# svohr/mixemt

Hardware: AMD Instinct MI355X
Metric: read x hap cells/sec through the EM iteration (EM iters/sec reported beside it as em_iters_per_s), 1000000 reads x 5408 haps in total, whole job (higher is better)
Workload: dtype f64

## Files before the change

### mixemt_amd/csrc/coded_kernels.hpp

```cpp
#ifndef MIXEMT_CODED_KERNELS_HPP
#define MIXEMT_CODED_KERNELS_HPP

#define ENC_THREADS 256
#define ENC_SLOTS 1024
#define ENC_MAX_CODES 256
#define ENC_MAX_WIDE 1024
#define ENC_WIDE_SLOTS 4096
#define ENC_EMPTY 0xFFFFFFFFFFFFFFFFull

__host__ __device__ __forceinline__ int rec_code_bytes(int nd, int ldc) { return nd > ENC_MAX_CODES ? 2 * ldc : ldc; }
__device__ __forceinline__ int rec_code_at(const uint8_t *codes, int h, bool wide) {
    return wide ? (int)reinterpret_cast<const uint16_t *>(codes)[h] : (int)codes[h];
}

template <int NCH, bool WIDE>
__device__ __forceinline__ void encode_one_row(int64_t r, const double *__restrict__ M, int64_t ldm, int H, int ldc,
                                               uint8_t *__restrict__ rec, int64_t rec_cap, int64_t *__restrict__ rec_off,
                                               int32_t *__restrict__ ndist, double *__restrict__ rowmax,
                                               unsigned long long *__restrict__ stats) {
    constexpr int NW = ENC_THREADS / 64;
    constexpr int SLOTS = WIDE ? ENC_WIDE_SLOTS : ENC_SLOTS;
    constexpr int MAXC = WIDE ? ENC_MAX_WIDE : ENC_MAX_CODES;
    constexpr int SPT = SLOTS / ENC_THREADS;
    __shared__ unsigned long long s_key[SLOTS];
// ... 212 lines not shown
                                               int64_t n_list = 0, const int32_t *__restrict__ nquad = nullptr, int vbid = -1,
                                               int vgrid = 0) {
    static_assert(NBUF >= 3, "codes NBUF - 1 rows ahead, tables NBUF - 2");
    constexpr int NW = THREADS / 64;
    constexpr int AUX = NT ? 2 : 0;
    __shared__ double s_tbl[NBUF][ENC_MAX_CODES];
    __shared__ __attribute__((aligned(16))) double red[NBUF][NW];
    const int t = threadIdx.x, lane = t & 63, wv = t >> 6;
    const int nword = ldc >> 2;
    const int64_t bid = vbid >= 0 ? (int64_t)vbid : (int64_t)blockIdx.x, grid = vbid >= 0 ? (int64_t)vgrid : (int64_t)gridDim.x;
    const row_deal deal(row_list != nullptr ? n_list : R, bid, grid);
    const int voff = t * 4;
    int last_w = t + (NCH - 1) * THREADS;
    if (last_w > nword - 1) last_w = nword - 1;
    const int voff_last = last_w * 4;
    const bool tbl_thread = (THREADS <= ENC_MAX_CODES) || t < ENC_MAX_CODES;
    const int tslot = t & (ENC_MAX_CODES - 1);
    typedef unsigned int u2v __attribute__((ext_vector_type(2)));
    __shared__ int s_chk[2];
    if constexpr (CHECK) {
        if (t == 0) s_chk[0] = s_chk[1] = 0;
        __syncthreads();
    }
    auto list_row = [&](int64_t e) -> int64_t {
        int64_t r = wide_rows[e];
        if constexpr (CHECK) {
            if (r < 0 || r >= R || (e > 0 && wide_rows[e - 1] >= r)) {
                s_chk[1] = 1;
                r = -1;
            }
        }
        return r;
    };
    auto list_nd = [&](int64_t r) -> int {
        if (r < 0) return 0;
        int nd = ndist[r];
        if constexpr (CHECK) {
            if (nd <= ENC_MAX_CODES) {
                s_chk[1] = 1;
                nd = 0;
            }
        }
        return nd;
    };

    __shared__ long long s_off[2][THREADS];
    __shared__ double s_wr[2][THREADS];
    __shared__ int s_nd[2][THREADS];
    auto fetch_meta = [&](int half, int64_t q0) {
        const int64_t q = q0 + t;
        int64_t r = deal.row(q);
        bool struck = false;
        if (row_list != nullptr) {
            const int64_t e = r;
            r = row_list[e];
            if constexpr (CHECK) {
                if (r < 0 || r >= R || (e > 0 && row_list[e - 1] >= r)) {
                    s_chk[1] = 1;
                    r = 0;
                    struck = true;
                }
            }
        }
        int nd = ndist[r];
        if (nd > ENC_MAX_CODES) {
            if constexpr (CHECK) {
                if (row_list != nullptr) s_chk[1] = 1;
                else if (deal.live(q)) atomicAdd(&s_chk[0], 1);
            }
            nd = 0;
        }
        if constexpr (CHECK) {
            if (row_list != nullptr && !struck && (nd <= 0 || nquad[r] != 0)) {
                s_chk[1] = 1;
                struck = true;
            }
        }
        if (struck) nd = 0;
        s_off[half][t] = rec_off[r];
        s_nd[half][t] = nd;
        s_wr[half][t] = (deal.live(q) && nd > 0) ? (w != nullptr ? w[r] : 1.0) : 0.0;
    };

    unsigned int cw[NBUF][NCH];
    double tring[NBUF];
    int pre_off_lo, pre_off_hi, pre_nd;
    double pre_wr;
    auto read_meta = [&](int64_t q_load, int64_t q_weight) {
        const int half = (int)((q_load / THREADS) & 1), idx = (int)(q_load % THREADS);
        const long long off = s_off[half][idx];
        pre_nd = __builtin_amdgcn_readfirstlane(s_nd[half][idx]);
        pre_off_hi = __builtin_amdgcn_readfirstlane((int)(off >> 32));
        pre_off_lo = __builtin_amdgcn_readfirstlane((int)off);
        pre_wr = s_wr[(q_weight / THREADS) & 1][q_weight % THREADS];
    };
    auto load_row = [&](unsigned int(&cws)[NCH], double &tbl_entry) {
        const int nd = pre_nd;
        const uint8_t *base = rec + (((long long)pre_off_hi << 32) | (unsigned int)pre_off_lo);
        const auto rs = __builtin_amdgcn_make_buffer_rsrc(const_cast<uint8_t *>(base), 0, ldc, 0x00020000);
#pragma unroll
        for (int k = 0; k < NCH - 1; ++k) cws[k] = __builtin_amdgcn_raw_buffer_load_b32(rs, voff, k * THREADS * 4, AUX);
        cws[NCH - 1] = __builtin_amdgcn_raw_buffer_load_b32(rs, voff_last, 0, AUX);
        if (tbl_thread) {
            const auto rt = __builtin_amdgcn_make_buffer_rsrc(const_cast<uint8_t *>(base + ldc), 0, nd * 8, 0x00020000);
            const u2v v = __builtin_amdgcn_raw_buffer_load_b64(rt, tslot * 8, 0, AUX);
            tbl_entry = __hiloint2double((int)v.y, (int)v.x);
        }
    };

    const unsigned int three = 3;
    auto entry_off = [&](unsigned int word, auto E) -> unsigned int {
        constexpr int e = decltype(E)::value;
        unsigned int r;
        if constexpr (e == 0) asm("v_lshlrev_b32_sdwa %0, %1, %2 dst_sel:DWORD dst_unused:UNUSED_PAD src0_sel:DWORD src1_sel:BYTE_0" : "=v"(r) : "v"(three), "v"(word));
        else if constexpr (e == 1) asm("v_lshlrev_b32_sdwa %0, %1, %2 dst_sel:DWORD dst_unused:UNUSED_PAD src0_sel:DWORD src1_sel:BYTE_1" : "=v"(r) : "v"(three), "v"(word));
        else if constexpr (e == 2) asm("v_lshlrev_b32_sdwa %0, %1, %2 dst_sel:DWORD dst_unused:UNUSED_PAD src0_sel:DWORD src1_sel:BYTE_2" : "=v"(r) : "v"(three), "v"(word));
        else asm("v_lshlrev_b32_sdwa %0, %1, %2 dst_sel:DWORD dst_unused:UNUSED_PAD src0_sel:DWORD src1_sel:BYTE_3" : "=v"(r) : "v"(three), "v"(word));
        return r;
    };
    auto lookup = [&](const char *tb, unsigned int word, auto E) -> double {
        return *reinterpret_cast<const double *>(tb + entry_off(word, E));
    };
    using E0 = std::integral_constant<int, 0>;
    using E1 = std::integral_constant<int, 1>;
    using E2 = std::integral_constant<int, 2>;
    using E3 = std::integral_constant<int, 3>;

    double v[NCH][4];
    auto lookup_row = [&](const char *tb, const unsigned int(&cws)[NCH]) {
#pragma unroll
        for (int k = 0; k < NCH; ++k) {
            v[k][0] = lookup(tb, cws[k], E0{});
            v[k][1] = lookup(tb, cws[k], E1{});
            v[k][2] = lookup(tb, cws[k], E2{});
            v[k][3] = lookup(tb, cws[k], E3{});
        }
    };

    auto step = [&](auto J, int64_t q) {
        constexpr int j = decltype(J)::value;
        constexpr int jn = (j + 1) % NBUF, jl = (j + NBUF - 1) % NBUF;
        if constexpr (!RESIDENT) {
            if ((q % THREADS) == 0) fetch_meta((int)((q / THREADS + 1) & 1), q + THREADS);
        }
        load_row(cw[jl], tring[jl]);
        const double wr = pre_wr;
        double s4[4] = {0.0, 0.0, 0.0, 0.0};
#pragma unroll
        for (int k = 0; k < NCH; ++k)
#pragma unroll
            for (int e = 0; e < 4; ++e) s4[e] = fma(v[k][e], p[k][e], s4[e]);
        double s = (s4[0] + s4[1]) + (s4[2] + s4[3]);
        __builtin_amdgcn_s_setprio(1);
        s = wave_sum_lane63(s);
        if (lane == 63) red[j][wv] = s;
        if (tbl_thread) s_tbl[jn][tslot] = tring[jn];
        __syncthreads();
        read_meta(q + NBUF, q + 1);
        static_assert(NW == 4, "four wave sums");
        typedef double d2v __attribute__((ext_vector_type(2)));
        const d2v ra = *reinterpret_cast<const d2v *>(&red[j][0]), rb = *reinterpret_cast<const d2v *>(&red[j][2]);
        const double cf = readlane_f64(weight_over_norm(wr, (ra.x + ra.y) + (rb.x + rb.y)), 0);
        __builtin_amdgcn_s_setprio(0);
        const char *tbn = reinterpret_cast<const char *>(&s_tbl[jn][0]);
        auto upd = [&](int k, auto E) {
            constexpr int e = decltype(E)::value;
            acc[k][e] = fma(cf, v[k][e], acc[k][e]);
            asm volatile("" : "+v"(acc[k][e]));
            v[k][e] = lookup(tbn, cw[jn][k], E);
        };
#pragma unroll
        for (int k = 0; k < NCH; ++k) {
            upd(k, E0{});
            upd(k, E1{});
            upd(k, E2{});
            upd(k, E3{});
        }
    };

    const int64_t nq_w = (n_wide > bid) ? (n_wide - bid + grid - 1) / grid : 0;
    const bool wide_fetch = WIDE_PREFETCH && nq_w > 0 && (!RESIDENT || !meta_ready);
    int64_t w_row = -1;
    if (wide_fetch && t < nq_w) w_row = list_row(bid + (int64_t)t * grid);
    long long w_off = 0;
    int w_nd = CHECK ? -1 : 0;
    double w_wr = 0.0;

    if (deal.nq > 0) {
        if (!RESIDENT || !meta_ready) {
            __syncthreads();
            fetch_meta(0, 0);
            if constexpr (RESIDENT) fetch_meta(1, THREADS);
        }
        __syncthreads();
#pragma unroll
        for (int j = 0; j < NBUF - 1; ++j) {
            read_meta(j, 0);
            load_row(cw[j], tring[j]);
        }
        if (tbl_thread) s_tbl[0][tslot] = tring[0];
        __syncthreads();
        read_meta(NBUF - 1, 0);
        lookup_row(reinterpret_cast<const char *>(&s_tbl[0][0]), cw[0]);
        if (w_row >= 0) {
            w_off = rec_off[w_row];
            w_nd = ndist[w_row];
            w_wr = (w != nullptr) ? w[w_row] : 1.0;
        }
        for (int64_t q = 0; q < deal.nq; q += NBUF) {
            step(std::integral_constant<int, 0>{}, q);
            step(std::integral_constant<int, 1>{}, q + 1);
            step(std::integral_constant<int, 2>{}, q + 2);
            if constexpr (NBUF > 3) step(std::integral_constant<int, 3>{}, q + 3);
            if constexpr (NBUF > 4) step(std::integral_constant<int, 4>{}, q + 4);
            if constexpr (NBUF > 5) step(std::integral_constant<int, 5>{}, q + 5);
            static_assert(NBUF <= 6, "unrolled by hand");
        }
    }

    else if (w_row >= 0) {
        w_off = rec_off[w_row];
        w_nd = ndist[w_row];
        w_wr = (w != nullptr) ? w[w_row] : 1.0;
    }

    if (nq_w > 0) {
        __shared__ double s_wide[ENC_MAX_WIDE];
        __shared__ long long s_woff[THREADS];
        __shared__ double s_wwr[THREADS];
        __shared__ int s_wnd[THREADS];
        constexpr int TPT = ENC_MAX_WIDE / THREADS;
        const int voff8 = t * 8;
        const int voff8_last = last_w * 8;
        for (int64_t q0 = 0; q0 < nq_w; q0 += THREADS) {
            if (q0 == 0 && wide_fetch) {
                __syncthreads();
                if constexpr (CHECK) {
                    if (w_nd >= 0 && w_nd <= ENC_MAX_CODES) s_chk[1] = 1;
                    if (w_nd <= ENC_MAX_CODES) {
                        w_nd = 0;
                        w_wr = 0.0;
                    }
                }
                s_woff[t] = w_off;
                s_wnd[t] = w_nd;
                s_wwr[t] = w_wr;
            } else if (q0 > 0 || !RESIDENT || !meta_ready || nq_w > THREADS) {
                __syncthreads();
                const int64_t q = q0 + t;
                if (q < nq_w) {
                    const int64_t r = list_row(bid + q * grid);
                    const int nd = list_nd(r);
                    s_woff[t] = (r >= 0) ? rec_off[r] : 0;
                    s_wnd[t] = nd;
                    s_wwr[t] = (nd > 0) ? ((w != nullptr) ? w[r] : 1.0) : 0.0;
                }
            }
            __syncthreads();
            const int n_here = (int)((nq_w - q0) < THREADS ? (nq_w - q0) : THREADS);
            u2v cwa[NCH], cwb[NCH], cwc[NCH];
            double tna[TPT], tnb[TPT], tnc[TPT];
            auto fetch_wide = [&](int i, u2v(&cwn)[NCH], double(&tn)[TPT]) {
                const long long off = s_woff[i];
                const int nd = __builtin_amdgcn_readfirstlane(s_wnd[i]);
                const uint8_t *base = rec + (((long long)__builtin_amdgcn_readfirstlane((int)(off >> 32)) << 32) |
                                             (unsigned int)__builtin_amdgcn_readfirstlane((int)off));
                const auto rs = __builtin_amdgcn_make_buffer_rsrc(const_cast<uint8_t *>(base), 0, 2 * ldc, 0x00020000);
#pragma unroll
                for (int k = 0; k < NCH - 1; ++k) cwn[k] = __builtin_amdgcn_raw_buffer_load_b64(rs, voff8, k * THREADS * 8, AUX);
                cwn[NCH - 1] = __builtin_amdgcn_raw_buffer_load_b64(rs, voff8_last, 0, AUX);
                const auto rt = __builtin_amdgcn_make_buffer_rsrc(const_cast<uint8_t *>(base + 2 * ldc), 0, nd * 8, 0x00020000);
#pragma unroll
                for (int j = 0; j < TPT; ++j) {
                    const u2v x = __builtin_amdgcn_raw_buffer_load_b64(rt, (t + j * THREADS) * 8, 0, AUX);
                    tn[j] = __hiloint2double((int)x.y, (int)x.x);
                }
            };
            auto process_wide = [&](int i, const u2v(&cwn)[NCH], const double(&tn)[TPT]) {
                const double wr = s_wwr[i];
#pragma unroll
                for (int j = 0; j < TPT; ++j) s_wide[t + j * THREADS] = tn[j];
                __syncthreads();
                const char *tb = reinterpret_cast<const char *>(&s_wide[0]);
                double s4[4] = {0.0, 0.0, 0.0, 0.0};
#pragma unroll
                for (int k = 0; k < NCH; ++k) {
                    v[k][0] = *reinterpret_cast<const double *>(tb + ((cwn[k].x & 0xffffu) << 3));
                    v[k][1] = *reinterpret_cast<const double *>(tb + ((cwn[k].x >> 16) << 3));
                    v[k][2] = *reinterpret_cast<const double *>(tb + ((cwn[k].y & 0xffffu) << 3));
                    v[k][3] = *reinterpret_cast<const double *>(tb + ((cwn[k].y >> 16) << 3));
                }
#pragma unroll
                for (int k = 0; k < NCH; ++k)
#pragma unroll
                    for (int e = 0; e < 4; ++e) s4[e] = fma(v[k][e], p[k][e], s4[e]);
                double s = (s4[0] + s4[1]) + (s4[2] + s4[3]);
                s = wave_sum_lane63(s);
                if (lane == 63) red[0][wv] = s;
                __syncthreads();
                static_assert(NW == 4, "four wave sums");
                const double cf = readlane_f64(weight_over_norm(wr, (red[0][0] + red[0][1]) + (red[0][2] + red[0][3])), 0);
#pragma unroll
                for (int k = 0; k < NCH; ++k)
#pragma unroll
                    for (int e = 0; e < 4; ++e) acc[k][e] = fma(cf, v[k][e], acc[k][e]);
            };
            fetch_wide(0, cwa, tna);
// ... 180 lines not shown
```

### mixemt_amd/csrc/common.hpp

```cpp
#ifndef MIXEMT_COMMON_HPP
#define MIXEMT_COMMON_HPP

typedef double d2 __attribute__((ext_vector_type(2)));

#define MXM_MAX_WG 1024
#define MXM_MAX_BT 4

struct mxm_slots {
    int s[MXM_MAX_BT];
};
#define MXM_LINEAR_MIN_H 65

static thread_local char g_err[512] = "";

static int fail(int code, const char *fmt, const char *a = "", long long b = 0, long long c = 0) {
    snprintf(g_err, sizeof(g_err), fmt, a, b, c);
    return code;
}
#define HIP_TRY(expr)                                                                        \
    do {                                                                                     \
        hipError_t e_ = (expr);                                                              \
        if (e_ != hipSuccess) return fail(-2, "HIP error: %s (line %lld)", hipGetErrorString(e_), __LINE__); \
    } while (0)

#define MXM_MAX_DEVICES 64
static std::atomic<int> g_num_cu[MXM_MAX_DEVICES];
static int num_cu() {
    int dev = 0;
    if (hipGetDevice(&dev) != hipSuccess) return 256;
    const bool cached = dev >= 0 && dev < MXM_MAX_DEVICES;
    if (cached) {
        const int have = g_num_cu[dev].load(std::memory_order_relaxed);
        if (have > 0) return have;
    }
    hipDeviceProp_t prop;
    if (hipGetDeviceProperties(&prop, dev) != hipSuccess) return 256;
    const int n = prop.multiProcessorCount > 0 ? prop.multiProcessorCount : 256;
    if (cached) g_num_cu[dev].store(n, std::memory_order_relaxed);
    return n;
}

__device__ __forceinline__ double wave_sum(double v) {
#pragma unroll
    for (int off = 32; off > 0; off >>= 1) v += __shfl_xor(v, off, 64);
    return v;
}
__device__ __forceinline__ double wave_max(double v) {
#pragma unroll
    for (int off = 32; off > 0; off >>= 1) v = fmax(v, __shfl_xor(v, off, 64));
    return v;
}

template <int THREADS, bool IS_MAX>
__device__ __forceinline__ double block_reduce(double v, double *scratch) {
    constexpr int NW = THREADS / 64;
    v = IS_MAX ? wave_max(v) : wave_sum(v);
    __syncthreads();
    if ((threadIdx.x & 63) == 0) scratch[threadIdx.x >> 6] = v;
    __syncthreads();
    double r = scratch[0];
#pragma unroll
    for (int i = 1; i < NW; ++i) r = IS_MAX ? fmax(r, scratch[i]) : r + scratch[i];
    return r;
}

template <int CTRL>
__device__ __forceinline__ double dpp_mov_f64(double v) {
    int lo = __double2loint(v), hi = __double2hiint(v);
    lo = __builtin_amdgcn_mov_dpp(lo, CTRL, 0xf, 0xf, true);
    hi = __builtin_amdgcn_mov_dpp(hi, CTRL, 0xf, 0xf, true);
    return __hiloint2double(hi, lo);
}
__device__ __forceinline__ double readlane_f64(double v, int src_lane) {
    const int lo = __builtin_amdgcn_readlane(__double2loint(v), src_lane);
    const int hi = __builtin_amdgcn_readlane(__double2hiint(v), src_lane);
    return __hiloint2double(hi, lo);
}
template <int CTRL, int ROW_MASK>
__device__ __forceinline__ double dpp_mov_old_f64(double old, double v) {
    int lo = __double2loint(v), hi = __double2hiint(v);
    lo = __builtin_amdgcn_update_dpp(__double2loint(old), lo, CTRL, ROW_MASK, 0xf, false);
    hi = __builtin_amdgcn_update_dpp(__double2hiint(old), hi, CTRL, ROW_MASK, 0xf, false);
    return __hiloint2double(hi, lo);
}
__device__ __forceinline__ double wave_sum_lane63(double v) {
    v += dpp_mov_f64<0xB1>(v);
    v += dpp_mov_f64<0x4E>(v);
    v += dpp_mov_f64<0x141>(v);
    v += dpp_mov_f64<0x140>(v);
    v += dpp_mov_old_f64<0x142, 0xA>(0.0, v);
    v += dpp_mov_old_f64<0x143, 0xC>(0.0, v);
    return v;
}
__device__ __forceinline__ double swap32_add(double x, double y) {
    typedef unsigned int u2s __attribute__((ext_vector_type(2)));
    const u2s lo = __builtin_amdgcn_permlane32_swap((unsigned)__double2loint(x), (unsigned)__double2loint(y), false, false);
    const u2s hi = __builtin_amdgcn_permlane32_swap((unsigned)__double2hiint(x), (unsigned)__double2hiint(y), false, false);
    return __hiloint2double((int)hi.x, (int)lo.x) + __hiloint2double((int)hi.y, (int)lo.y);
}
__device__ __forceinline__ double swap16_add(double x, double y) {
    typedef unsigned int u2s __attribute__((ext_vector_type(2)));
    const u2s lo = __builtin_amdgcn_permlane16_swap((unsigned)__double2loint(x), (unsigned)__double2loint(y), false, false);
    const u2s hi = __builtin_amdgcn_permlane16_swap((unsigned)__double2hiint(x), (unsigned)__double2hiint(y), false, false);
    return __hiloint2double((int)hi.x, (int)lo.x) + __hiloint2double((int)hi.y, (int)lo.y);
}
__device__ __forceinline__ double wave_sum3_by_row(double a, double b, double c) {
    const double ab = swap32_add(a, b);
    const double cc = swap32_add(c, c);
    double v = swap16_add(ab, cc);
    v += dpp_mov_f64<0xB1>(v);
    v += dpp_mov_f64<0x4E>(v);
    v += dpp_mov_f64<0x141>(v);
    v += dpp_mov_f64<0x140>(v);
    return v;
}
__device__ __forceinline__ double wave_max_lane63(double v) {
    v = fmax(v, dpp_mov_f64<0xB1>(v));
    v = fmax(v, dpp_mov_f64<0x4E>(v));
    v = fmax(v, dpp_mov_f64<0x141>(v));
    v = fmax(v, dpp_mov_f64<0x140>(v));
    v = fmax(v, dpp_mov_old_f64<0x142, 0xA>(v, v));
    v = fmax(v, dpp_mov_old_f64<0x143, 0xC>(v, v));
    return v;
}

__device__ __forceinline__ int wave_min_lane63_i32(int v) {
    v = min(v, __builtin_amdgcn_mov_dpp(v, 0xB1, 0xf, 0xf, true));
    v = min(v, __builtin_amdgcn_mov_dpp(v, 0x4E, 0xf, 0xf, true));
    v = min(v, __builtin_amdgcn_mov_dpp(v, 0x141, 0xf, 0xf, true));
    v = min(v, __builtin_amdgcn_mov_dpp(v, 0x140, 0xf, 0xf, true));
    v = min(v, __builtin_amdgcn_update_dpp(v, v, 0x142, 0xA, 0xf, false));
    v = min(v, __builtin_amdgcn_update_dpp(v, v, 0x143, 0xC, 0xf, false));
    return v;
}

__device__ __forceinline__ int wave_inclusive_scan_i32(int v) {
    v += __builtin_amdgcn_update_dpp(0, v, 0x111, 0xf, 0xf, false);
    v += __builtin_amdgcn_update_dpp(0, v, 0x112, 0xf, 0xf, false);
    v += __builtin_amdgcn_update_dpp(0, v, 0x114, 0xf, 0xf, false);
    v += __builtin_amdgcn_update_dpp(0, v, 0x118, 0xf, 0xf, false);
    v += __builtin_amdgcn_update_dpp(0, v, 0x142, 0xa, 0xf, false);
    v += __builtin_amdgcn_update_dpp(0, v, 0x143, 0xc, 0xf, false);
    return v;
}

__device__ __forceinline__ double weight_over_norm(double wr, double z) {
    if (z > 0.0) return wr / z;
    return (wr != 0.0) ? __builtin_nan("") : 0.0;
}

template <int NW, int N>
__device__ __forceinline__ void group_ratio_to_sgpr(const double *red, int lane, double num, double (&c)[N]) {
    static_assert(NW == 4 || NW == 8 || NW == 16, "waves per workgroup");
    static_assert(N * NW <= 64, "one partial per lane");
    double v = red[lane < N * NW ? lane : 0];
    v += dpp_mov_f64<0xB1>(v);
    v += dpp_mov_f64<0x4E>(v);
    if constexpr (NW >= 8) v += dpp_mov_f64<0x141>(v);
    if constexpr (NW == 16) v += dpp_mov_f64<0x140>(v);
    v = weight_over_norm(num, v);
#pragma unroll
    for (int g = 0; g < N; ++g) c[g] = readlane_f64(v, g * NW);
}

__device__ __forceinline__ double logaddexp_f64(double a, double b) {
    if (a == b) return a + 0.693147180559945309417232121458176568;
    double d = a - b;
    if (d > 0) return a + log1p(exp(-d));
    if (d <= 0) return b + log1p(exp(d));
    return d;
}

template <int E>
__device__ __forceinline__ unsigned int code_byte_x8(unsigned int word) {
    const unsigned int three = 3;
    unsigned int r;
    if constexpr (E == 0) asm("v_lshlrev_b32_sdwa %0, %1, %2 dst_sel:DWORD dst_unused:UNUSED_PAD src0_sel:DWORD src1_sel:BYTE_0" : "=v"(r) : "v"(three), "v"(word));
    else if constexpr (E == 1) asm("v_lshlrev_b32_sdwa %0, %1, %2 dst_sel:DWORD dst_unused:UNUSED_PAD src0_sel:DWORD src1_sel:BYTE_1" : "=v"(r) : "v"(three), "v"(word));
    else if constexpr (E == 2) asm("v_lshlrev_b32_sdwa %0, %1, %2 dst_sel:DWORD dst_unused:UNUSED_PAD src0_sel:DWORD src1_sel:BYTE_2" : "=v"(r) : "v"(three), "v"(word));
    else asm("v_lshlrev_b32_sdwa %0, %1, %2 dst_sel:DWORD dst_unused:UNUSED_PAD src0_sel:DWORD src1_sel:BYTE_3" : "=v"(r) : "v"(three), "v"(word));
    return r;
}

struct row_deal {
    int64_t nq;
    int64_t bid, grid;
    __device__ explicit row_deal(int64_t R) : row_deal(R, blockIdx.x, gridDim.x) {}
    __device__ row_deal(int64_t R, int64_t b, int64_t g) : nq((R - b + g - 1) / g), bid(b), grid(g) {}
    __device__ bool live(int64_t q) const { return q < nq; }
    __device__ int64_t row(int64_t q) const { return bid + (q < nq ? q : nq - 1) * grid; }
};

#endif
```

### mixemt_amd/csrc/quad_kernels.hpp

```cpp
#ifndef MIXEMT_QUAD_KERNELS_HPP
#define MIXEMT_QUAD_KERNELS_HPP

#define QUAD_MAX 256
#define QUAD_CODE_BYTES 2048
#define QUAD_HASH 1024
#define QUAD_THREADS 256
#define QUAD_CHUNK 65536ull

typedef unsigned int quad_u2 __attribute__((ext_vector_type(2)));
typedef unsigned int quad_u4 __attribute__((ext_vector_type(4)));
typedef double quad_d2 __attribute__((ext_vector_type(2)));

__global__ __launch_bounds__(QUAD_THREADS) void quad_encode_kernel(const uint8_t *__restrict__ rec,
                                                                   const int64_t *__restrict__ rec_off,
                                                                   const int32_t *__restrict__ ndist, int ldc, int H, int64_t R,
                                                                   uint8_t *__restrict__ qrec, unsigned long long qcap,
                                                                   int64_t *__restrict__ qoff, int32_t *__restrict__ nquad,
                                                                   unsigned long long *__restrict__ stats) {
#ifndef QUAD_RANK_BY_COUNT
#define QUAD_RANK_BY_COUNT 0
#endif
    __shared__ unsigned long long s_tab[QUAD_HASH];
    __shared__ int s_cnt[QUAD_RANK_BY_COUNT ? QUAD_HASH : 1];
    __shared__ int s_kcnt[QUAD_RANK_BY_COUNT ? QUAD_MAX : 1];
// ... 424 lines not shown
            nquad[first + lane] = nq_v;
            qoff[first + lane] = at_v;
        }
        nd_v = nd_v2;
        off_v = off_v2;
    }
}

__global__ __launch_bounds__(256) void quad_validate_kernel(const int32_t *__restrict__ ndist, const int32_t *__restrict__ nquad,
                                                           int64_t R, const int64_t *__restrict__ quad_rows, int64_t n_quad,
                                                           const int64_t *__restrict__ byte_rows, int64_t n_byte,
                                                           unsigned long long *__restrict__ out) {
    const int64_t stride = (int64_t)gridDim.x * 256;
    bool bad = false;
    for (int64_t e = (int64_t)blockIdx.x * 256 + threadIdx.x; e < n_quad; e += stride) {
        const int64_t r = quad_rows[e];
        if (r < 0 || r >= R || (e > 0 && quad_rows[e - 1] >= r)) bad = true;
        else bad = bad || nquad[r] < 1 || nquad[r] > QUAD_MAX || ndist[r] < 1 || ndist[r] > ENC_MAX_CODES;
    }
    for (int64_t e = (int64_t)blockIdx.x * 256 + threadIdx.x; e < n_byte; e += stride) {
        const int64_t r = byte_rows[e];
        if (r < 0 || r >= R || (e > 0 && byte_rows[e - 1] >= r)) bad = true;
        else bad = bad || nquad[r] != 0 || ndist[r] < 1 || ndist[r] > ENC_MAX_CODES;
    }
    if (bad) out[1] = 1ull;
}

#define QLIST_THREADS 256
#define QLIST_PER_THREAD 16
#define QLIST_CHUNK (QLIST_THREADS * QLIST_PER_THREAD)
__device__ __forceinline__ int quad_row_class(const int32_t *__restrict__ ndist, const int32_t *__restrict__ nquad, int64_t r) {
    if (nquad[r] > 0) return 1;
    const int nd = ndist[r];
    return (nd > 0 && nd <= ENC_MAX_CODES) ? 2 : 0;
}
__global__ __launch_bounds__(QLIST_THREADS) void quad_list_count_kernel(const int32_t *__restrict__ ndist,
                                                                       const int32_t *__restrict__ nquad, int64_t R,
                                                                       long long *__restrict__ chunk_counts ) {
    __shared__ int s_c[2];
    if (threadIdx.x < 2) s_c[threadIdx.x] = 0;
    __syncthreads();
    const int64_t r0 = (int64_t)blockIdx.x * QLIST_CHUNK + (int64_t)threadIdx.x * QLIST_PER_THREAD;
    int nq = 0, nb = 0;
    for (int i = 0; i < QLIST_PER_THREAD; ++i) {
        const int64_t r = r0 + i;
        if (r < R) {
            const int c = quad_row_class(ndist, nquad, r);
            nq += (c == 1);
            nb += (c == 2);
        }
    }
    if (nq) atomicAdd(&s_c[0], nq);
    if (nb) atomicAdd(&s_c[1], nb);
    __syncthreads();
    if (threadIdx.x < 2) chunk_counts[2 * blockIdx.x + threadIdx.x] = s_c[threadIdx.x];
}
__global__ __launch_bounds__(QLIST_THREADS) void quad_list_scan_kernel(long long *__restrict__ chunk_counts, int64_t nchunk,
                                                                      long long *__restrict__ counts) {
    __shared__ long long s_sum[2][QLIST_THREADS];
    const int t = threadIdx.x;
    const int64_t per = (nchunk + QLIST_THREADS - 1) / QLIST_THREADS;
    const int64_t lo = (int64_t)t * per, hi = (lo + per < nchunk) ? lo + per : nchunk;
    long long a = 0, b = 0;
    for (int64_t i = lo; i < hi; ++i) {
        a += chunk_counts[2 * i];
        b += chunk_counts[2 * i + 1];
    }
    s_sum[0][t] = a;
    s_sum[1][t] = b;
    __syncthreads();
    if (t == 0) {
        long long ra = 0, rb = 0;
        for (int i = 0; i < QLIST_THREADS; ++i) {
            const long long xa = s_sum[0][i], xb = s_sum[1][i];
            s_sum[0][i] = ra;
            s_sum[1][i] = rb;
            ra += xa;
            rb += xb;
        }
        counts[0] = ra;
        counts[1] = rb;
    }
    __syncthreads();
    a = s_sum[0][t];
    b = s_sum[1][t];
    for (int64_t i = lo; i < hi; ++i) {
        const long long xa = chunk_counts[2 * i], xb = chunk_counts[2 * i + 1];
        chunk_counts[2 * i] = a;
        chunk_counts[2 * i + 1] = b;
        a += xa;
        b += xb;
    }
}
__global__ __launch_bounds__(QLIST_THREADS) void quad_list_fill_kernel(const int32_t *__restrict__ ndist,
                                                                      const int32_t *__restrict__ nquad, int64_t R,
                                                                      const long long *__restrict__ chunk_base,
                                                                      int64_t *__restrict__ quad_rows,
                                                                      int64_t *__restrict__ byte_rows) {
    __shared__ int s_q[QLIST_THREADS], s_b[QLIST_THREADS];
    const int t = threadIdx.x;
    const int64_t r0 = (int64_t)blockIdx.x * QLIST_CHUNK + (int64_t)t * QLIST_PER_THREAD;
    int cls[QLIST_PER_THREAD];
    int nq = 0, nb = 0;
#pragma unroll
    for (int i = 0; i < QLIST_PER_THREAD; ++i) {
        const int64_t r = r0 + i;
        cls[i] = (r < R) ? quad_row_class(ndist, nquad, r) : 0;
        nq += (cls[i] == 1);
        nb += (cls[i] == 2);
    }
    s_q[t] = nq;
    s_b[t] = nb;
    __syncthreads();
    if (t == 0) {
        int rq = 0, rb = 0;
        for (int i = 0; i < QLIST_THREADS; ++i) {
            const int xq = s_q[i], xb = s_b[i];
            s_q[i] = rq;
            s_b[i] = rb;
            rq += xq;
            rb += xb;
        }
    }
    __syncthreads();
    long long oq = chunk_base[2 * blockIdx.x] + s_q[t], ob = chunk_base[2 * blockIdx.x + 1] + s_b[t];
#pragma unroll
    for (int i = 0; i < QLIST_PER_THREAD; ++i) {
        if (cls[i] == 1) quad_rows[oq++] = r0 + i;
        else if (cls[i] == 2) byte_rows[ob++] = r0 + i;
    }
}

template <int B>
__device__ __forceinline__ unsigned int quad_byte_x16(unsigned int word) {
    const unsigned int four = 4;
    unsigned int r;
    if constexpr (B == 0) asm("v_lshlrev_b32_sdwa %0, %1, %2 dst_sel:DWORD dst_unused:UNUSED_PAD src0_sel:DWORD src1_sel:BYTE_0" : "=v"(r) : "v"(four), "v"(word));
    else if constexpr (B == 1) asm("v_lshlrev_b32_sdwa %0, %1, %2 dst_sel:DWORD dst_unused:UNUSED_PAD src0_sel:DWORD src1_sel:BYTE_1" : "=v"(r) : "v"(four), "v"(word));
    else if constexpr (B == 2) asm("v_lshlrev_b32_sdwa %0, %1, %2 dst_sel:DWORD dst_unused:UNUSED_PAD src0_sel:DWORD src1_sel:BYTE_2" : "=v"(r) : "v"(four), "v"(word));
    else asm("v_lshlrev_b32_sdwa %0, %1, %2 dst_sel:DWORD dst_unused:UNUSED_PAD src0_sel:DWORD src1_sel:BYTE_3" : "=v"(r) : "v"(four), "v"(word));
    return r;
}
template <int B>
__device__ __forceinline__ unsigned int quad_byte_x32(unsigned int word) {
    const unsigned int five = 5;
    unsigned int r;
    if constexpr (B == 0) asm("v_lshlrev_b32_sdwa %0, %1, %2 dst_sel:DWORD dst_unused:UNUSED_PAD src0_sel:DWORD src1_sel:BYTE_0" : "=v"(r) : "v"(five), "v"(word));
    else if constexpr (B == 1) asm("v_lshlrev_b32_sdwa %0, %1, %2 dst_sel:DWORD dst_unused:UNUSED_PAD src0_sel:DWORD src1_sel:BYTE_1" : "=v"(r) : "v"(five), "v"(word));
    else if constexpr (B == 2) asm("v_lshlrev_b32_sdwa %0, %1, %2 dst_sel:DWORD dst_unused:UNUSED_PAD src0_sel:DWORD src1_sel:BYTE_2" : "=v"(r) : "v"(five), "v"(word));
    else asm("v_lshlrev_b32_sdwa %0, %1, %2 dst_sel:DWORD dst_unused:UNUSED_PAD src0_sel:DWORD src1_sel:BYTE_3" : "=v"(r) : "v"(five), "v"(word));
    return r;
}

template <int NCH, int NBUF, bool NT>
__device__ __forceinline__ void quad_row_pass(const uint8_t *__restrict__ qrec, const int64_t *__restrict__ qoff,
                                              const int32_t *__restrict__ nquad, const int64_t *__restrict__ quad_rows,
                                              int64_t n_rows, int64_t R, const double *__restrict__ w,
                                              const double (&p)[NCH][4], double (&acc)[NCH][4], int *fault, int vbid = -1,
                                              int vgrid = 0) {
    static_assert(NBUF >= 3 && NBUF <= 6, "codes NBUF - 1 rows ahead; unrolled by hand");
    static_assert(NCH >= 1 && NCH <= 8, "eight code bytes per thread");
    constexpr int THREADS = QUAD_THREADS, NW = THREADS / 64, AUX = NT ? 2 : 0;
    __shared__ __attribute__((aligned(16))) double s_tbl[NBUF][QUAD_MAX * 4];
    __shared__ __attribute__((aligned(16))) double red[NBUF][NW];
    __shared__ long long s_off[2][THREADS];
    __shared__ double s_wr[2][THREADS];
    __shared__ int s_nd[2][THREADS];
    __shared__ int s_fault;
    const int t = threadIdx.x, lane = t & 63, wv = t >> 6;
    const row_deal deal(n_rows, vbid >= 0 ? (int64_t)vbid : (int64_t)blockIdx.x, vbid >= 0 ? (int64_t)vgrid : (int64_t)gridDim.x);
    if (t == 0) s_fault = 0;

    auto fetch_meta = [&](int half, int64_t q0) {
        const int64_t q = q0 + t;
        const int64_t e = deal.row(q);
        int64_t r = quad_rows[e];
        int nd = 0;
        if (r < 0 || r >= R || (e > 0 && quad_rows[e - 1] >= r)) {
            s_fault = 1;
            r = -1;
        } else {
            nd = nquad[r];
            if (nd <= 0 || nd > QUAD_MAX) {
                s_fault = 1;
                nd = 0;
            }
        }
        s_off[half][t] = (nd > 0) ? qoff[r] : 0;
        s_nd[half][t] = nd;
        s_wr[half][t] = (deal.live(q) && nd > 0) ? (w != nullptr ? w[r] : 1.0) : 0.0;
    };
    quad_u2 cw[NBUF];
    double tring[NBUF][4];
    int pre_off_lo, pre_off_hi, pre_nd;
    double pre_wr;
    auto read_meta = [&](int64_t q_load, int64_t q_weight) {
        const int half = (int)((q_load / THREADS) & 1), idx = (int)(q_load % THREADS);
        const long long off = s_off[half][idx];
        pre_nd = __builtin_amdgcn_readfirstlane(s_nd[half][idx]);
        pre_off_hi = __builtin_amdgcn_readfirstlane((int)(off >> 32));
        pre_off_lo = __builtin_amdgcn_readfirstlane((int)off);
        pre_wr = s_wr[(q_weight / THREADS) & 1][q_weight % THREADS];
    };
    auto load_row = [&](auto SLOT) {
        constexpr int slot = decltype(SLOT)::value;
        const int nd = pre_nd;
        const uint8_t *base = qrec + (((long long)pre_off_hi << 32) | (unsigned int)pre_off_lo);
        const auto rs = __builtin_amdgcn_make_buffer_rsrc(const_cast<uint8_t *>(base), 0, nd > 0 ? QUAD_CODE_BYTES : 0, 0x00020000);
        cw[slot] = __builtin_amdgcn_raw_buffer_load_b64(rs, t * 8, 0, AUX);
        const auto rt = __builtin_amdgcn_make_buffer_rsrc(const_cast<uint8_t *>(base + QUAD_CODE_BYTES), 0, nd * 32, 0x00020000);
        const quad_u4 a = __builtin_amdgcn_raw_buffer_load_b128(rt, t * 32, 0, AUX);
        const quad_u4 b = __builtin_amdgcn_raw_buffer_load_b128(rt, t * 32, 16, AUX);
        tring[slot][0] = __hiloint2double((int)a.y, (int)a.x);
        tring[slot][1] = __hiloint2double((int)a.w, (int)a.z);
        tring[slot][2] = __hiloint2double((int)b.y, (int)b.x);
        tring[slot][3] = __hiloint2double((int)b.w, (int)b.z);
    };
#ifndef QUAD_SPLIT_TABLE
#define QUAD_SPLIT_TABLE 1
#endif
    auto publish = [&](auto SLOT) {
        constexpr int slot = decltype(SLOT)::value;
#if QUAD_SPLIT_TABLE
        *reinterpret_cast<quad_d2 *>(&s_tbl[slot][t * 2]) = quad_d2{tring[slot][0], tring[slot][1]};
        *reinterpret_cast<quad_d2 *>(&s_tbl[slot][QUAD_MAX * 2 + t * 2]) = quad_d2{tring[slot][2], tring[slot][3]};
#else
        quad_d2 *dst = reinterpret_cast<quad_d2 *>(&s_tbl[slot][t * 4]);
        dst[0] = quad_d2{tring[slot][0], tring[slot][1]};
        dst[1] = quad_d2{tring[slot][2], tring[slot][3]};
#endif
    };
    double v[NCH][4];
    auto lookup_quad = [&](const char *tb, auto K, const quad_u2 &c) {
        constexpr int k = decltype(K)::value;
        unsigned int off;
#if QUAD_SPLIT_TABLE
        if constexpr (k < 4) off = quad_byte_x16<k>(c.x);
        else off = quad_byte_x16<k - 4>(c.y);
        const quad_d2 a = *reinterpret_cast<const quad_d2 *>(tb + off), b = *reinterpret_cast<const quad_d2 *>(tb + off + QUAD_MAX * 16);
#else
        if constexpr (k < 4) off = quad_byte_x32<k>(c.x);
        else off = quad_byte_x32<k - 4>(c.y);
        const quad_d2 a = *reinterpret_cast<const quad_d2 *>(tb + off), b = *reinterpret_cast<const quad_d2 *>(tb + off + 16);
#endif
        v[k][0] = a.x;
        v[k][1] = a.y;
        v[k][2] = b.x;
        v[k][3] = b.y;
    };
    auto lookup_row = [&](const char *tb, const quad_u2 &c) {
        lookup_quad(tb, std::integral_constant<int, 0>{}, c);
        if constexpr (NCH > 1) lookup_quad(tb, std::integral_constant<int, 1>{}, c);
        if constexpr (NCH > 2) lookup_quad(tb, std::integral_constant<int, 2>{}, c);
        if constexpr (NCH > 3) lookup_quad(tb, std::integral_constant<int, 3>{}, c);
        if constexpr (NCH > 4) lookup_quad(tb, std::integral_constant<int, 4>{}, c);
        if constexpr (NCH > 5) lookup_quad(tb, std::integral_constant<int, 5>{}, c);
        if constexpr (NCH > 6) lookup_quad(tb, std::integral_constant<int, 6>{}, c);
        if constexpr (NCH > 7) lookup_quad(tb, std::integral_constant<int, 7>{}, c);
    };

    auto step = [&](auto J, int64_t q) {
        constexpr int j = decltype(J)::value;
        constexpr int jn = (j + 1) % NBUF, jl = (j + NBUF - 1) % NBUF;
        if ((q % THREADS) == 0) fetch_meta((int)((q / THREADS + 1) & 1), q + THREADS);
        load_row(std::integral_constant<int, jl>{});
        const double wr = pre_wr;
        double s4[4] = {0.0, 0.0, 0.0, 0.0};
#pragma unroll
        for (int k = 0; k < NCH; ++k)
#pragma unroll
            for (int e = 0; e < 4; ++e) s4[e] = fma(v[k][e], p[k][e], s4[e]);
        double s = (s4[0] + s4[1]) + (s4[2] + s4[3]);
        __builtin_amdgcn_s_setprio(1);
        s = wave_sum_lane63(s);
        if (lane == 63) red[j][wv] = s;
        publish(std::integral_constant<int, jn>{});
        __syncthreads();
        read_meta(q + NBUF, q + 1);
        static_assert(NW == 4, "four wave sums");
        const quad_d2 ra = *reinterpret_cast<const quad_d2 *>(&red[j][0]), rb = *reinterpret_cast<const quad_d2 *>(&red[j][2]);
        const double cf = readlane_f64(weight_over_norm(wr, (ra.x + ra.y) + (rb.x + rb.y)), 0);
        __builtin_amdgcn_s_setprio(0);
        const char *tbn = reinterpret_cast<const char *>(&s_tbl[jn][0]);
        auto upd = [&](auto K) {
            constexpr int k = decltype(K)::value;
            if constexpr (k < NCH) {
#pragma unroll
                for (int e = 0; e < 4; ++e) {
                    acc[k][e] = fma(cf, v[k][e], acc[k][e]);
                    asm volatile("" : "+v"(acc[k][e]));
                }
                lookup_quad(tbn, K, cw[jn]);
            }
        };
        upd(std::integral_constant<int, 0>{});
        upd(std::integral_constant<int, 1>{});
        upd(std::integral_constant<int, 2>{});
        upd(std::integral_constant<int, 3>{});
        upd(std::integral_constant<int, 4>{});
        upd(std::integral_constant<int, 5>{});
        upd(std::integral_constant<int, 6>{});
        upd(std::integral_constant<int, 7>{});
    };

    if (deal.nq > 0) {
        __syncthreads();
        fetch_meta(0, 0);
        __syncthreads();
        read_meta(0, 0);
        load_row(std::integral_constant<int, 0>{});
        read_meta(1, 0);
        load_row(std::integral_constant<int, 1>{});
        if constexpr (NBUF > 3) {
            read_meta(2, 0);
            load_row(std::integral_constant<int, 2>{});
        }
        if constexpr (NBUF > 4) {
            read_meta(3, 0);
            load_row(std::integral_constant<int, 3>{});
        }
        if constexpr (NBUF > 5) {
            read_meta(4, 0);
            load_row(std::integral_constant<int, 4>{});
        }
        publish(std::integral_constant<int, 0>{});
        __syncthreads();
        read_meta(NBUF - 1, 0);
        lookup_row(reinterpret_cast<const char *>(&s_tbl[0][0]), cw[0]);
        for (int64_t q = 0; q < deal.nq; q += NBUF) {
            step(std::integral_constant<int, 0>{}, q);
            step(std::integral_constant<int, 1>{}, q + 1);
            step(std::integral_constant<int, 2>{}, q + 2);
            if constexpr (NBUF > 3) step(std::integral_constant<int, 3>{}, q + 3);
            if constexpr (NBUF > 4) step(std::integral_constant<int, 4>{}, q + 4);
            if constexpr (NBUF > 5) step(std::integral_constant<int, 5>{}, q + 5);
        }
    }
    __syncthreads();
    *fault = s_fault;
}

template <int NCH, int NBUF>
__global__ __launch_bounds__(QUAD_THREADS, 2) void em_iter_quad_kernel(
    const uint8_t *__restrict__ qrec, const int64_t *__restrict__ qoff, const int32_t *__restrict__ nquad,
    const int64_t *__restrict__ quad_rows, int64_t n_rows, int64_t R, const double *__restrict__ w,
    const double *__restrict__ props, int H, double *__restrict__ partial, int64_t ldpart, int part_row0,
    const mxm_em_state *__restrict__ state, int run) {
    if (state != nullptr && state[run].done != 0) return;
    const int t = threadIdx.x;
    props += (int64_t)run * H;
    double p[NCH][4], acc[NCH][4];
#pragma unroll
    for (int k = 0; k < NCH; ++k) {
#pragma unroll
        for (int e = 0; e < 4; ++e) {
            const int c = 4 * (t + k * QUAD_THREADS) + e;
            p[k][e] = (c < H) ? props[c] : 0.0;
            acc[k][e] = 0.0;
        }
    }
    int fault = 0;
    quad_row_pass<NCH, NBUF, true>(qrec, qoff, nquad, quad_rows, n_rows, R, w, p, acc, &fault);
    const int64_t row = (int64_t)part_row0 + blockIdx.x;
    if (t == 0) {
        int *out = reinterpret_cast<int *>(partial + (int64_t)MXM_MAX_WG * ldpart) + 2 * row;
        out[0] = 0;
        out[1] = fault;
    }
    double *dst = partial + row * ldpart;
#pragma unroll
    for (int k = 0; k < NCH; ++k) {
        const int c = 4 * (t + k * QUAD_THREADS);
#pragma unroll
        for (int e = 0; e < 4; ++e)
            if (c + e < H) dst[c + e] = acc[k][e];
    }
}

template <int NCH, int NBUF>
__global__ __launch_bounds__(QUAD_THREADS, 2) void em_iter_quad_coded_kernel(
    const uint8_t *__restrict__ rec, const int64_t *__restrict__ rec_off, const int32_t *__restrict__ ndist, int ldc,
    const int64_t *__restrict__ wide_rows, int64_t n_wide, const int64_t *__restrict__ byte_rows, int64_t n_byte_rows,
    const uint8_t *__restrict__ qrec, const int64_t *__restrict__ qoff, const int32_t *__restrict__ nquad,
    const int64_t *__restrict__ quad_rows, int64_t n_quad_rows, int64_t R, const double *__restrict__ w,
    const double *__restrict__ props, int H, double *__restrict__ partial, int64_t ldpart, int nwg_left,
    const mxm_em_state *__restrict__ state, int run) {
    if (state != nullptr && state[run].done != 0) return;
    const int t = threadIdx.x;
    props += (int64_t)run * H;
    double p[NCH][4], acc[NCH][4];
#pragma unroll
    for (int k = 0; k < NCH; ++k) {
#pragma unroll
        for (int e = 0; e < 4; ++e) {
            const int c = 4 * (t + k * QUAD_THREADS) + e;
            p[k][e] = (c < H) ? props[c] : 0.0;
            acc[k][e] = 0.0;
        }
    }
    const int nwg_quad = (int)gridDim.x - nwg_left;
    int chk[2] = {0, 0};
    int64_t prow;
    if ((int)blockIdx.x < nwg_left) {
        bool meta_ready = false;
        coded_row_pass<QUAD_THREADS, NCH, NBUF, true, false, true, true>(rec, rec_off, ndist, ldc, w, wide_rows, n_wide, R, p, acc,
                                                                         meta_ready, chk, byte_rows, n_byte_rows, nquad,
                                                                         (int)blockIdx.x, nwg_left);
        prow = (int64_t)nwg_quad + blockIdx.x;
    } else {
        quad_row_pass<NCH, NBUF, true>(qrec, qoff, nquad, quad_rows, n_quad_rows, R, w, p, acc, &chk[1],
                                       (int)blockIdx.x - nwg_left, nwg_quad);
        prow = (int64_t)blockIdx.x - nwg_left;
    }
    if (t == 0) {
        int *out = reinterpret_cast<int *>(partial + (int64_t)MXM_MAX_WG * ldpart) + 2 * prow;
        out[0] = chk[0];
        out[1] = chk[1];
    }
    double *dst = partial + prow * ldpart;
#pragma unroll
    for (int k = 0; k < NCH; ++k) {
        const int c = 4 * (t + k * QUAD_THREADS);
#pragma unroll
        for (int e = 0; e < 4; ++e)
            if (c + e < H) dst[c + e] = acc[k][e];
    }
}

__global__ __launch_bounds__(QUAD_THREADS, 2) void diag_stream_quads_kernel(const uint8_t *__restrict__ qrec,
                                                                           const int64_t *__restrict__ qoff,
                                                                           const int32_t *__restrict__ nquad,
                                                                           const int64_t *__restrict__ quad_rows, int64_t n_rows,
                                                                           int64_t R, unsigned int *__restrict__ sink) {
    constexpr int NBUF = 4, THREADS = QUAD_THREADS;
    static_assert(THREADS % NBUF == 0, "a block of steps is a whole number of rounds");
    __shared__ long long s_off[2][THREADS];
    __shared__ int s_nd[2][THREADS];
    const int t = threadIdx.x;
    const row_deal deal(n_rows);
    if (deal.nq <= 0) return;
    quad_u2 x[NBUF];
    quad_u4 ya[NBUF], yb[NBUF];
    unsigned int acc = 0;
    auto fetch_meta = [&](int half, int64_t q0) {
        const int64_t q = q0 + t;
        const int64_t r = quad_rows[deal.row(q)];
        const bool ok = deal.live(q) && r >= 0 && r < R;
        const int nd = ok ? nquad[r] : 0;
        s_off[half][t] = nd > 0 && nd <= QUAD_MAX ? qoff[r] : 0;
        s_nd[half][t] = nd > 0 && nd <= QUAD_MAX ? nd : 0;
    };
    auto load_rec = [&](int slot, int64_t q) {
        const int half = (int)((q / THREADS) & 1), idx = (int)(q % THREADS);
        const long long off = s_off[half][idx];
        const int nd = __builtin_amdgcn_readfirstlane(s_nd[half][idx]);
        const int off_hi = __builtin_amdgcn_readfirstlane((int)(off >> 32)), off_lo = __builtin_amdgcn_readfirstlane((int)off);
        const uint8_t *base = qrec + (((long long)off_hi << 32) | (unsigned int)off_lo);
        const auto rs = __builtin_amdgcn_make_buffer_rsrc(const_cast<uint8_t *>(base), 0, nd > 0 ? QUAD_CODE_BYTES : 0, 0x00020000);
        x[slot] = __builtin_amdgcn_raw_buffer_load_b64(rs, t * 8, 0, 2);
        const auto rt = __builtin_amdgcn_make_buffer_rsrc(const_cast<uint8_t *>(base + QUAD_CODE_BYTES), 0, nd * 32, 0x00020000);
        ya[slot] = __builtin_amdgcn_raw_buffer_load_b128(rt, t * 32, 0, 2);
        yb[slot] = __builtin_amdgcn_raw_buffer_load_b128(rt, t * 32, 16, 2);
    };
    fetch_meta(0, 0);
    __syncthreads();
#pragma unroll
    for (int j = 0; j < NBUF - 1; ++j) load_rec(j, j);
    const int64_t nblk = (deal.nq + THREADS - 1) / THREADS;
    for (int64_t b = 0; b < nblk; ++b) {
        __syncthreads();
        fetch_meta((int)((b + 1) & 1), (b + 1) * THREADS);
        __syncthreads();
        for (int i = 0; i < THREADS; i += NBUF) {
#pragma unroll
            for (int j = 0; j < NBUF; ++j) {
                load_rec((j + NBUF - 1) % NBUF, b * THREADS + i + j + NBUF - 1);
                acc ^= x[j].x ^ x[j].y ^ ya[j].x ^ ya[j].w ^ yb[j].y ^ yb[j].z;
            }
        }
    }
    if (acc == 0x9e3779b9u) sink[0] = acc;
}

#endif
```

Baseline: 881.3 billion.

## Skip dead last chunk per wave and rotate quad thread roles across workgroups

Adds a per-wave compile-time specialization so waves whose last column chunk lies entirely beyond H skip that chunk's FMAs and table lookups in the quad row pass. Workgroups are also given a rotated thread-to-column mapping based on a block-id bit, so the partially live tail chunk lands on different waves in alternating blocks and the load is spread across SIMDs. The wave reduction is replaced by a variant that carries the DPP temporary forward rather than zero-filling, which is meant to trim dependent adds while keeping a correct lane-63 result. Costs are extra code size from instantiating two loop bodies, plus some added complexity in the thread index math.

Result: no change. 874.4 billion (-0.8%).

```diff
diff --git a/mixemt_amd/csrc/coded_kernels.hpp b/mixemt_amd/csrc/coded_kernels.hpp
--- a/mixemt_amd/csrc/coded_kernels.hpp
+++ b/mixemt_amd/csrc/coded_kernels.hpp
@@ -388,7 +388,7 @@
             for (int e = 0; e < 4; ++e) s4[e] = fma(v[k][e], p[k][e], s4[e]);
         double s = (s4[0] + s4[1]) + (s4[2] + s4[3]);
         __builtin_amdgcn_s_setprio(1);
-        s = wave_sum_lane63(s);
+        s = wave_sum_lane63_only(s);
         if (lane == 63) red[j][wv] = s;
         if (tbl_thread) s_tbl[jn][tslot] = tring[jn];
         __syncthreads();
diff --git a/mixemt_amd/csrc/common.hpp b/mixemt_amd/csrc/common.hpp
--- a/mixemt_amd/csrc/common.hpp
+++ b/mixemt_amd/csrc/common.hpp
@@ -92,6 +92,17 @@
     v += dpp_mov_old_f64<0x143, 0xC>(0.0, v);
     return v;
 }
+__device__ __forceinline__ double wave_sum_lane63_only(double v) {
+    v += dpp_mov_f64<0xB1>(v);
+    v += dpp_mov_f64<0x4E>(v);
+    v += dpp_mov_f64<0x141>(v);
+    double tmp = dpp_mov_f64<0x140>(v);
+    v += tmp;
+    tmp = dpp_mov_old_f64<0x142, 0xA>(tmp, v);
+    v += tmp;
+    tmp = dpp_mov_old_f64<0x143, 0xC>(tmp, v);
+    return v + tmp;
+}
 __device__ __forceinline__ double swap32_add(double x, double y) {
     typedef unsigned int u2s __attribute__((ext_vector_type(2)));
     const u2s lo = __builtin_amdgcn_permlane32_swap((unsigned)__double2loint(x), (unsigned)__double2loint(y), false, false);
diff --git a/mixemt_amd/csrc/quad_kernels.hpp b/mixemt_amd/csrc/quad_kernels.hpp
--- a/mixemt_amd/csrc/quad_kernels.hpp
+++ b/mixemt_amd/csrc/quad_kernels.hpp
@@ -600,12 +600,20 @@
     return r;
 }
 
+#ifndef QUAD_ROLE_BIT
+#define QUAD_ROLE_BIT 0
+#endif
+__device__ __forceinline__ int quad_pass_thread(int wg) {
+    const int turn = QUAD_ROLE_BIT < 0 ? 0 : (wg >> (QUAD_ROLE_BIT < 0 ? 0 : QUAD_ROLE_BIT)) & 1;
+    return ((int)threadIdx.x + (QUAD_THREADS / 2) * turn) & (QUAD_THREADS - 1);
+}
+
 template <int NCH, int NBUF, bool NT>
 __device__ __forceinline__ void quad_row_pass(const uint8_t *__restrict__ qrec, const int64_t *__restrict__ qoff,
                                               const int32_t *__restrict__ nquad, const int64_t *__restrict__ quad_rows,
                                               int64_t n_rows, int64_t R, const double *__restrict__ w,
-                                              const double (&p)[NCH][4], double (&acc)[NCH][4], int *fault, int vbid = -1,
-                                              int vgrid = 0) {
+                                              const double (&p)[NCH][4], double (&acc)[NCH][4], int *fault, int t, int H,
+                                              int vbid = -1, int vgrid = 0) {
     static_assert(NBUF >= 3 && NBUF <= 6, "codes NBUF - 1 rows ahead; unrolled by hand");
     static_assert(NCH >= 1 && NCH <= 8, "eight code bytes per thread");
     constexpr int THREADS = QUAD_THREADS, NW = THREADS / 64, AUX = NT ? 2 : 0;
@@ -615,7 +623,8 @@
     __shared__ double s_wr[2][THREADS];
     __shared__ int s_nd[2][THREADS];
     __shared__ int s_fault;
-    const int t = threadIdx.x, lane = t & 63, wv = t >> 6;
+    const int lane = t & 63, wv = __builtin_amdgcn_readfirstlane(t >> 6);
+    const bool last_chunk_live = 4 * (THREADS * (NCH - 1) + 64 * wv) < H;
     const row_deal deal(n_rows, vbid >= 0 ? (int64_t)vbid : (int64_t)blockIdx.x, vbid >= 0 ? (int64_t)vgrid : (int64_t)gridDim.x);
     if (t == 0) s_fault = 0;
 
@@ -696,31 +705,32 @@
         v[k][2] = b.x;
         v[k][3] = b.y;
     };
-    auto lookup_row = [&](const char *tb, const quad_u2 &c) {
-        lookup_quad(tb, std::integral_constant<int, 0>{}, c);
-        if constexpr (NCH > 1) lookup_quad(tb, std::integral_constant<int, 1>{}, c);
-        if constexpr (NCH > 2) lookup_quad(tb, std::integral_constant<int, 2>{}, c);
-        if constexpr (NCH > 3) lookup_quad(tb, std::integral_constant<int, 3>{}, c);
-        if constexpr (NCH > 4) lookup_quad(tb, std::integral_constant<int, 4>{}, c);
-        if constexpr (NCH > 5) lookup_quad(tb, std::integral_constant<int, 5>{}, c);
-        if constexpr (NCH > 6) lookup_quad(tb, std::integral_constant<int, 6>{}, c);
-        if constexpr (NCH > 7) lookup_quad(tb, std::integral_constant<int, 7>{}, c);
-    };
-
-    auto step = [&](auto J, int64_t q) {
-        constexpr int j = decltype(J)::value;
+    auto lookup_row = [&](const char *tb, const quad_u2 &c, auto NL) {
+        constexpr int nl = decltype(NL)::value;
+        if constexpr (nl > 0) lookup_quad(tb, std::integral_constant<int, 0>{}, c);
+        if constexpr (nl > 1) lookup_quad(tb, std::integral_constant<int, 1>{}, c);
+        if constexpr (nl > 2) lookup_quad(tb, std::integral_constant<int, 2>{}, c);
+        if constexpr (nl > 3) lookup_quad(tb, std::integral_constant<int, 3>{}, c);
+        if constexpr (nl > 4) lookup_quad(tb, std::integral_constant<int, 4>{}, c);
+        if constexpr (nl > 5) lookup_quad(tb, std::integral_constant<int, 5>{}, c);
+        if constexpr (nl > 6) lookup_quad(tb, std::integral_constant<int, 6>{}, c);
+        if constexpr (nl > 7) lookup_quad(tb, std::integral_constant<int, 7>{}, c);
+    };
+
+    auto step = [&](auto J, auto NL, int64_t q) {
+        constexpr int j = decltype(J)::value, nl = decltype(NL)::value;
         constexpr int jn = (j + 1) % NBUF, jl = (j + NBUF - 1) % NBUF;
         if ((q % THREADS) == 0) fetch_meta((int)((q / THREADS + 1) & 1), q + THREADS);
         load_row(std::integral_constant<int, jl>{});
         const double wr = pre_wr;
         double s4[4] = {0.0, 0.0, 0.0, 0.0};
 #pragma unroll
-        for (int k = 0; k < NCH; ++k)
+        for (int k = 0; k < nl; ++k)
 #pragma unroll
             for (int e = 0; e < 4; ++e) s4[e] = fma(v[k][e], p[k][e], s4[e]);
         double s = (s4[0] + s4[1]) + (s4[2] + s4[3]);
         __builtin_amdgcn_s_setprio(1);
-        s = wave_sum_lane63(s);
+        s = wave_sum_lane63_only(s);
         if (lane == 63) red[j][wv] = s;
         publish(std::integral_constant<int, jn>{});
         __syncthreads();
@@ -732,7 +742,7 @@
         const char *tbn = reinterpret_cast<const char *>(&s_tbl[jn][0]);
         auto upd = [&](auto K) {
             constexpr int k = decltype(K)::value;
-            if constexpr (k < NCH) {
+            if constexpr (k < nl) {
 #pragma unroll
                 for (int e = 0; e < 4; ++e) {
                     acc[k][e] = fma(cf, v[k][e], acc[k][e]);
@@ -774,15 +784,19 @@
         publish(std::integral_constant<int, 0>{});
         __syncthreads();
         read_meta(NBUF - 1, 0);
-        lookup_row(reinterpret_cast<const char *>(&s_tbl[0][0]), cw[0]);
-        for (int64_t q = 0; q < deal.nq; q += NBUF) {
-            step(std::integral_constant<int, 0>{}, q);
-            step(std::integral_constant<int, 1>{}, q + 1);
-            step(std::integral_constant<int, 2>{}, q + 2);
-            if constexpr (NBUF > 3) step(std::integral_constant<int, 3>{}, q + 3);
-            if constexpr (NBUF > 4) step(std::integral_constant<int, 4>{}, q + 4);
-            if constexpr (NBUF > 5) step(std::integral_constant<int, 5>{}, q + 5);
-        }
+        auto rows = [&](auto NL) {
+            lookup_row(reinterpret_cast<const char *>(&s_tbl[0][0]), cw[0], NL);
+            for (int64_t q = 0; q < deal.nq; q += NBUF) {
+                step(std::integral_constant<int, 0>{}, NL, q);
+                step(std::integral_constant<int, 1>{}, NL, q + 1);
+                step(std::integral_constant<int, 2>{}, NL, q + 2);
+                if constexpr (NBUF > 3) step(std::integral_constant<int, 3>{}, NL, q + 3);
+                if constexpr (NBUF > 4) step(std::integral_constant<int, 4>{}, NL, q + 4);
+                if constexpr (NBUF > 5) step(std::integral_constant<int, 5>{}, NL, q + 5);
+            }
+        };
+        if (last_chunk_live) rows(std::integral_constant<int, NCH>{});
+        else rows(std::integral_constant<int, NCH - 1>{});
     }
     __syncthreads();
     *fault = s_fault;
@@ -795,7 +809,7 @@
     const double *__restrict__ props, int H, double *__restrict__ partial, int64_t ldpart, int part_row0,
     const mxm_em_state *__restrict__ state, int run) {
     if (state != nullptr && state[run].done != 0) return;
-    const int t = threadIdx.x;
+    const int t = quad_pass_thread((int)blockIdx.x);
     props += (int64_t)run * H;
     double p[NCH][4], acc[NCH][4];
 #pragma unroll
@@ -808,7 +822,7 @@
         }
     }
     int fault = 0;
-    quad_row_pass<NCH, NBUF, true>(qrec, qoff, nquad, quad_rows, n_rows, R, w, p, acc, &fault);
+    quad_row_pass<NCH, NBUF, true>(qrec, qoff, nquad, quad_rows, n_rows, R, w, p, acc, &fault, t, H);
     const int64_t row = (int64_t)part_row0 + blockIdx.x;
     if (t == 0) {
         int *out = reinterpret_cast<int *>(partial + (int64_t)MXM_MAX_WG * ldpart) + 2 * row;
@@ -834,7 +848,8 @@
     const double *__restrict__ props, int H, double *__restrict__ partial, int64_t ldpart, int nwg_left,
     const mxm_em_state *__restrict__ state, int run) {
     if (state != nullptr && state[run].done != 0) return;
-    const int t = threadIdx.x;
+    const int nwg_quad = (int)gridDim.x - nwg_left;
+    const int t = (int)blockIdx.x < nwg_left ? (int)threadIdx.x : quad_pass_thread((int)blockIdx.x);
     props += (int64_t)run * H;
     double p[NCH][4], acc[NCH][4];
 #pragma unroll
@@ -846,7 +861,6 @@
             acc[k][e] = 0.0;
         }
     }
-    const int nwg_quad = (int)gridDim.x - nwg_left;
     int chk[2] = {0, 0};
     int64_t prow;
     if ((int)blockIdx.x < nwg_left) {
@@ -856,7 +870,7 @@
                                                                          (int)blockIdx.x, nwg_left);
         prow = (int64_t)nwg_quad + blockIdx.x;
     } else {
-        quad_row_pass<NCH, NBUF, true>(qrec, qoff, nquad, quad_rows, n_quad_rows, R, w, p, acc, &chk[1],
+        quad_row_pass<NCH, NBUF, true>(qrec, qoff, nquad, quad_rows, n_quad_rows, R, w, p, acc, &chk[1], t, H,
                                        (int)blockIdx.x - nwg_left, nwg_quad);
         prow = (int64_t)blockIdx.x - nwg_left;
     }
@@ -866,9 +880,11 @@
         out[1] = chk[1];
     }
     double *dst = partial + prow * ldpart;
+    int ts = t;
+    asm volatile("" : "+v"(ts));
 #pragma unroll
     for (int k = 0; k < NCH; ++k) {
-        const int c = 4 * (t + k * QUAD_THREADS);
+        const int c = 4 * (ts + k * QUAD_THREADS);
 #pragma unroll
         for (int e = 0; e < 4; ++e)
             if (c + e < H) dst[c + e] = acc[k][e];
```
